# harukaki/brl

Hardware: AMD Instinct MI355X
Metric: env-steps/sec at num_envs=8192, 32-step rollout, 1/2/4/8 MI355X (higher is better)
Workload: dtype u8; 1 GPU; configs[1]: num_envs=8192 num_steps=32 random-policy rollout + DDS reward (fused kernel) + last_obs + GAE scan; num_envs_per_gpu=8192, num_steps=32, lut_len=100000, env_steps_per_macro_step=1, transition_buffers_in_rotation=3, device_warmup=3328 untimed steps (80 ms) before the --warmup steps: steady-state clocks, parallelism=env-shard x1, no collective

## Files before the change

brl_amd/build.py:

```python
from __future__ import annotations

import os
import shutil
import subprocess
import sys

PKG = os.path.dirname(os.path.abspath(__file__))
INCLUDE = os.path.join(os.path.dirname(PKG), "include")
OUT = os.path.join(PKG, "lib", "libbrl_hip.so")
OBJ_DIR = os.path.join(PKG, "lib", "obj")

FLAGS = ["--offload-arch=gfx950", "-O3", "-ffp-contract=off", "-fPIC", "-std=c++17"]


def units():
    import glob
    return sorted(glob.glob(os.path.join(PKG, "csrc", "*.hip")))


def headers():
    import glob
    return sorted(glob.glob(os.path.join(PKG, "csrc", "*.hpp")) + glob.glob(os.path.join(INCLUDE, "*.h")))


def deps():
    return units() + headers()


def hipcc() -> str:
    for cand in (os.environ.get("HIPCC"), shutil.which("hipcc"), "/opt/rocm/bin/hipcc"):
        if cand and os.path.exists(cand):
            return cand
    raise RuntimeError("hipcc not found (set HIPCC)")


def needs_build() -> bool:
    if not os.path.exists(OUT):
        return True
    t = os.path.getmtime(OUT)
    return any(os.path.getmtime(d) > t for d in deps())


def build(force: bool = False, verbose: bool = False) -> str:
    if not (force or needs_build()):
        return OUT
    os.makedirs(OBJ_DIR, exist_ok=True)
    newest_header = max(os.path.getmtime(h) for h in headers())
    procs, objs = [], []
    for src in units():
        obj = os.path.join(OBJ_DIR, os.path.splitext(os.path.basename(src))[0] + ".o")
        objs.append(obj)
        if force or not os.path.exists(obj) or os.path.getmtime(obj) < max(os.path.getmtime(src), newest_header):
            cmd = [hipcc()] + FLAGS + ["-c", "-o", obj, src]
            if verbose:
                print(" ".join(cmd), flush=True)
            procs.append((cmd, subprocess.Popen(cmd)))
    for cmd, p in procs:
        if p.wait() != 0:
            raise subprocess.CalledProcessError(p.returncode, cmd)
    cmd = [hipcc(), "--offload-arch=gfx950", "-shared", "-fPIC", "-o", OUT] + objs
    if verbose:
        print(" ".join(cmd), flush=True)
    subprocess.check_call(cmd)
    return OUT


if __name__ == "__main__":
    print(build(force="--force" in sys.argv, verbose=True))
```

brl_amd/csrc/brl_rollout.hip:

```cpp
#include <hip/hip_runtime.h>
#include <math.h>
#include <stdint.h>
#include <stdio.h>
#include <stdlib.h>
#include <string.h>

#include "handle.hpp"
#include "policy_common.hpp"

struct RolloutArgs {
  uint64_t *state;
  int64_t n;
  int T;
  int substeps;
  uint32_t draw_base;
  float reward_scale;
  Rng g;
  uint64_t env_offset;
  LutRef lut;
  const float *neg_log_n;
  brl_transition out;
  uint8_t *last_obs;
  uint8_t *last_mask;
  unsigned long long *terminated_count;
// ... 795 lines not shown
    };
#pragma unroll
    for (int u = 0; u < HGP; u++) {
      if (wv + 4 * u >= hsteps) break;
#pragma unroll
      for (int nb = 0; nb < 3; nb++) acc[nb] = mma(hav[u], hbok[nb] ? hbv[u][nb] : zero8, acc[nb]);
    }
    if (hsteps > 4 * HGP) {
      const int64_t row0 = xcd_block((int64_t)blockIdx.x, (int64_t)gridDim.x) * 16;
      const int64_t arow = (row0 + r < A.n) ? row0 + r : A.n - 1;
      const uint16_t *ap = reinterpret_cast<const uint16_t *>(A.x.head_h) + arow * A.x.head_ldh + 8 * kq;
      for (int st = wv + 4 * HGP; st < hsteps; st += 4) {
        const pol_b16x8 a = *reinterpret_cast<const pol_b16x8 *>(ap + 32 * st);
#pragma unroll
        for (int nb = 0; nb < 3; nb++) {
          const pol_b16x8 b = *reinterpret_cast<const pol_b16x8 *>(reinterpret_cast<const uint16_t *>(A.x.head_w) +
                                                                   (int64_t)(hbok[nb] ? 16 * nb + r : 0) * A.x.head_hidden + 8 * kq + 32 * st);
          acc[nb] = mma(a, hbok[nb] ? b : zero8, acc[nb]);
        }
      }
    }
#pragma unroll
    for (int nb = 0; nb < 3; nb++)
#pragma unroll
      for (int q = 0; q < 4; q++) hd_red[wv][nb][q][lane] = acc[nb][q];
    __syncthreads();
    for (int e = tid; e < 16 * POL_HD; e += BLOCK_THREADS) {
      const int row = e / POL_HD, col = e - row * POL_HD;
      const int nb = col >> 4, c = col & 15, q = row & 3, rq = row >> 2;
      float v = A.x.head_b[col];
#pragma unroll
      for (int k = 0; k < 4; k++) v += hd_red[k][nb][q][16 * rq + c];
      hd_logits[row][col] = v;
    }
    __syncthreads();
  }
  const DevCtx cx = *A.ctx;
  const uint64_t legal = legal_mask(t);
  const uint64_t cand = (A.mode & 2) ? ALL_ACTIONS : legal;
  const bool owner = w.c.lane < K && w.valid;
  const int64_t otab = owner ? w.table : 0;
  float4 old_rw = make_float4(0.f, 0.f, 0.f, 0.f);
  uint32_t old_term = 0, val_raw = 0, actor_id = 0;
  if (A.o.rewards && !A.x.first) old_rw = reinterpret_cast<const float4 *>(A.o.rewards)[otab];
  if (A.o.terminated && !A.x.first) old_term = A.o.terminated[otab];
  const int in_fmt = HEADS ? 0 : A.x.in_fmt;
  if (A.x.value_out) {
    if (HEADS) val_raw = __float_as_uint(hd_logits[(int)(threadIdx.x >> 6) * K + (w.c.lane < K ? w.c.lane : 0)][BRL_NUM_ACTIONS]);
    else if (A.x.in_fmt == 0) val_raw = reinterpret_cast<const uint32_t *>(A.x.value_in)[otab * A.x.value_stride];
    else val_raw = reinterpret_cast<const uint16_t *>(A.x.value_in)[otab * A.x.value_stride];
  }
  if (A.x.last && A.x.reward_out) actor_id = (uint32_t)A.x.actor[otab];
  uint32_t u32 = 0;
  if (!(A.mode & 1)) {
    uint32_t r[4];
    const uint64_t env_id = cx.env_offset + (uint64_t)w.table;
    const uint32_t draw = A.draw + (A.draw_dev ? *A.draw_dev : 0u);
    philox4x32_10((uint32_t)env_id, draw >> 2, STREAM_ACTION, (uint32_t)(env_id >> 32), cx.g.k0, cx.g.k1, r);
    u32 = philox_word(r, draw);
  }
  float lp;
  const int act = HEADS ? categorical<K>(&hd_logits[0][0], (int64_t)((int)(threadIdx.x >> 6) * K + w.tl) * (POL_HD + 1), 0, w.valid, cand,
                                         A.mode, u32, w.c.lane, lp)
                        : categorical<K>(A.logits, (w.valid ? w.table : 0) * A.logits_stride, A.x.in_fmt, w.valid, cand, A.mode, u32,
                                         w.c.lane, lp);
  if (A.autoreset) auto_reset_clear(t);
  int hb = table_step(t, act);
  wave_or_hist<K>(w, hb);
  wave_lds_fence();
  uint32_t term = bits(t.sc, SC_TERM, 1);
  float4 rw = rewards_f32(t);
  if (A.autoreset) wave_reset<K>(w, t, w.valid && term, cx.g, cx.env_offset, cx.lut, t.bctr + 1u);
  int oseat = cur_seat(t);
  wave_emit<K>(w, A.n, oseat, vul_nibble(t, oseat), legal_mask(t), A.o.obs, A.o.mask, w.table0);
  if (A.x.obs_cast != nullptr) {
    const uint32_t pack = (uint32_t)oseat | (vul_nibble(t, oseat) << 2);
    const int esz = (A.x.obs_fmt == 0) ? 4 : 2;
#pragma unroll
    for (int j = 0; j < K; j++) {
      if (w.table0 + j < A.n) {
        const uint32_t p = __builtin_amdgcn_readlane(pack, j);
        emit_obs_row_cast(w.wimg + j * TABLE_BYTES, (int)(p & 3u), p >> 2,
                          reinterpret_cast<uint8_t *>(A.x.obs_cast) + (w.table0 + j) * BRL_OBS_SIZE * esz, A.x.obs_fmt, w.c);
      }
    }
  }
  uint32_t tacc = 0;
  if (w.c.lane < K && w.valid) {
    if (A.action) A.action[w.table] = act;
    if (A.log_prob) A.log_prob[w.table] = lp;
    float4 tot = rw;
    if (A.o.rewards) {
      if (!A.x.first) tot = make_float4(old_rw.x + rw.x, old_rw.y + rw.y, old_rw.z + rw.z, old_rw.w + rw.w);
      reinterpret_cast<float4 *>(A.o.rewards)[w.table] = tot;
    }
    tacc = term;
    if (A.o.terminated) {
      if (!A.x.first) tacc |= old_term;
      A.o.terminated[w.table] = (uint8_t)tacc;
    }
    if (A.o.current_player) A.o.current_player[w.table] = cur_player(t);
    if (A.x.value_out) A.x.value_out[w.table] = net_cvt(val_raw, in_fmt);
    if (A.x.last) {
      if (A.x.done_out) A.x.done_out[w.table] = (uint8_t)tacc;
      if (A.x.reward_out) {
        const int a = (int)(actor_id & 3u);
        const float r = (a == 0) ? tot.x : ((a == 1) ? tot.y : ((a == 2) ? tot.z : tot.w));
        A.x.reward_out[w.table] = r / A.x.reward_scale;
      }
    }
  }
  if (A.x.last && A.x.terminated_count) {
    __shared__ uint32_t tc_s[WAVES_PER_BLOCK];
    const uint64_t m = __ballot(tacc != 0u);
    if (w.c.lane == 0) tc_s[threadIdx.x >> 6] = (uint32_t)__popcll(m);
    __syncthreads();
    if (threadIdx.x == 0) {
      uint32_t c = 0;
#pragma unroll
      for (int k = 0; k < WAVES_PER_BLOCK; k++) c += tc_s[k];
      if (c) atomicAdd(reinterpret_cast<unsigned long long *>(A.x.terminated_count), (unsigned long long)c);
    }
  }
  wave_end<K>(w, t, A.state_out, A.n);
}

static inline bool aligned_to(const void *p, uintptr_t a) { return ((uintptr_t)p & (a - 1)) == 0; }
static bool transition_aligned(const brl_transition *o, const void *last_obs, const void *last_mask, const void *adv, const void *tgt) {
  return aligned_to(o->obs, 16) && aligned_to(o->legal_action_mask, 16) && aligned_to(o->action, 16) && aligned_to(o->value, 16) &&
         aligned_to(o->reward, 16) && aligned_to(o->log_prob, 16) && aligned_to(o->done, 4) && aligned_to(last_obs, 16) &&
         aligned_to(last_mask, 16) && aligned_to(adv, 16) && aligned_to(tgt, 16);
}

static bool every_column(const brl_transition *o) {
  return o->obs && o->legal_action_mask && o->done && o->action && o->value && o->reward && o->log_prob;
}
static RolloutArgs rollout_args(brl_handle *h, uint64_t *state, int64_t n, int num_steps, int substeps, uint32_t draw_base,
                                float reward_scale, const brl_transition *out, uint8_t *last_obs, uint8_t *last_mask,
                                int64_t *terminated_count) {
  RolloutArgs A;
  A.state = state; A.n = n; A.T = num_steps; A.substeps = substeps; A.draw_base = draw_base;
  A.reward_scale = reward_scale; A.g = rng_of(h); A.env_offset = h->env_offset; A.lut = lut_of(h);
  A.neg_log_n = h->neg_log_n; A.out = *out; A.terminated_count = (unsigned long long *)terminated_count;
  A.last_obs = last_obs; A.last_mask = last_mask;
  A.gae_last_val = nullptr; A.gae_gamma = 0.0f; A.gae_gamma_lambda = 0.0f; A.gae_adv = nullptr; A.gae_tgt = nullptr;
#ifdef BRL_TIMING
  A.debug = getenv("BRL_DEBUG") ? atoi(getenv("BRL_DEBUG")) : 0;
#else
  A.debug = 0;
#endif
  return A;
}

extern "C" int brl_rollout_random(brl_handle *h, uint64_t *state, int64_t n, int num_steps, int substeps,
                                  uint32_t draw_base, float reward_scale, const brl_transition *out,
                                  uint8_t *last_obs, uint8_t *last_mask, int64_t *terminated_count, void *stream) {
  COMMON(h, n);
  NEED(state && out, "state / out");
  NEED(aligned_to(state, 16) && transition_aligned(out, last_obs, last_mask, nullptr, nullptr),
       "output arrays must be 16-byte aligned (done: 4-byte)");
  NEED(num_steps >= 0, "num_steps");
  NEED(substeps >= 1 && substeps <= 16, "substeps");
  if (h->lut_len == 0) return fail(BRL_E_NOLUT, "brl_rollout_random auto-resets and needs a LUT%s", "");
  const RolloutArgs A = rollout_args(h, state, n, num_steps, substeps, draw_base, reward_scale, out, last_obs, last_mask, terminated_count);
  if (h->ws && h->fs && substeps == 1 && n % FS_TPB == 0 && every_column(out)) {
    const int pieces = (num_steps + FS_MAX_TOTAL - 1) / FS_MAX_TOTAL;
    int t0 = 0;
    for (int i = 0; i < pieces || (pieces == 0 && i == 0); i++) {
      const int len = (pieces > 0) ? (num_steps - t0 + (pieces - i) - 1) / (pieces - i) : 0;
      const int64_t rows = (int64_t)t0 * n;
      RolloutArgs P = A;
      P.T = len;
      P.draw_base = draw_base + (uint32_t)t0;
      P.out.obs = out->obs + rows * BRL_OBS_SIZE;
      P.out.legal_action_mask = out->legal_action_mask + rows * BRL_NUM_ACTIONS;
      P.out.done = out->done + rows;
      P.out.action = out->action + rows;
      P.out.value = out->value + rows;
      P.out.reward = out->reward + rows;
      P.out.log_prob = out->log_prob + rows;
      const bool last = (i + 1 >= pieces);
      P.last_obs = last ? last_obs : nullptr;
      P.last_mask = last ? last_mask : nullptr;
      hipLaunchKernelGGL(k_rollout_fs, dim3((unsigned)(n / FS_TPB)), dim3(FS_NW * 64), 0, (hipStream_t)stream, P);
      t0 += len;
    }
  } else if (h->ws && substeps <= WS_BATCH) {
    hipLaunchKernelGGL((k_rollout_ws<32, 12, 1>), dim3((unsigned)((n + 31) / 32)), dim3(12 * 64), 0, (hipStream_t)stream, A);
  } else {
    LAUNCH_K(h, k_rollout_random, n, stream, A);
    return BRL_OK;
  }
  HIP_TRY(hipGetLastError());
  return BRL_OK;
}

extern "C" int brl_rollout_random_gae(brl_handle *h, uint64_t *state, int64_t n, int num_steps, uint32_t draw_base,
                                      float reward_scale, const brl_transition *out, uint8_t *last_obs, uint8_t *last_mask,
                                      int64_t *terminated_count, const float *last_val, float gamma, float gamma_lambda,
                                      float *advantages, float *targets, void *stream) {
  COMMON(h, n);
  NEED(state && out && last_val && advantages && targets, "state / out / last_val / advantages / targets");
  NEED(num_steps >= 1, "num_steps");
  NEED(out->done && out->value && out->reward, "the done / value / reward columns");
  NEED(aligned_to(state, 16) && transition_aligned(out, last_obs, last_mask, advantages, targets),
       "output arrays must be 16-byte aligned (done: 4-byte)");
  if (h->lut_len == 0) return fail(BRL_E_NOLUT, "brl_rollout_random_gae auto-resets and needs a LUT%s", "");
  if (!(h->ws && h->fs && num_steps <= FS_MAX_TOTAL && n % FS_TPB == 0 && every_column(out))) {
    const int rc = brl_rollout_random(h, state, n, num_steps, 1, draw_base, reward_scale, out, last_obs, last_mask,
                                      terminated_count, stream);
    if (rc != BRL_OK) return rc;
    return brl_gae(h, out->done, out->value, out->reward, last_val, gamma, gamma_lambda, num_steps, n, advantages, targets, stream);
  }
  RolloutArgs A = rollout_args(h, state, n, num_steps, 1, draw_base, reward_scale, out, last_obs, last_mask, terminated_count);
  A.gae_last_val = last_val; A.gae_gamma = gamma; A.gae_gamma_lambda = gamma_lambda; A.gae_adv = advantages; A.gae_tgt = targets;
  hipLaunchKernelGGL(k_rollout_fs, dim3((unsigned)(n / FS_TPB)), dim3(FS_NW * 64), 0, (hipStream_t)stream, A);
  HIP_TRY(hipGetLastError());
  return BRL_OK;
}

static int policy_step_impl(brl_handle *h, const uint64_t *state_in, uint64_t *state_out, int64_t n,
                            const float *logits, int64_t logits_stride, int mode, const uint32_t *draw_dev, uint32_t draw,
                            int autoreset,
                            int32_t *action, float *log_prob, uint8_t *obs, uint8_t *mask, float *rewards_acc,
                            uint8_t *terminated_acc, int32_t *current_player, void *stream, const brl_macro_ext *ext = nullptr) {
  NEED(step_outputs_aligned(state_in, state_out, obs, rewards_acc, action, current_player) && ptr_aligned(log_prob, 4) &&
           ptr_aligned(draw_dev, 4), STEP_ALIGN_MSG);
  NEED(ext == nullptr || (ptr_aligned(ext->obs_cast, 16) && ptr_aligned(ext->value_out, 4) && ptr_aligned(ext->reward_out, 4) &&
                          ptr_aligned(ext->actor, 4) && ptr_aligned(ext->terminated_count, 8)),
       "ext: obs_cast not 16-byte aligned (value_out / reward_out / actor: 4-byte, terminated_count: 8-byte)");
  COMMON(h, n);
  const bool heads = ext != nullptr && (ext->head_h != nullptr || ext->head_part != nullptr);
  NEED(state_in && state_out && (logits || heads), "NULL state / logits");
  NEED(mode >= 0 && mode <= 3, "mode");
  NEED(heads || logits_stride >= BRL_NUM_ACTIONS, "logits_stride");
  if (autoreset && h->lut_len == 0) return fail(BRL_E_NOLUT, "auto-reset needs a LUT%s", "");
  PolicyArgs A;
  A.state_in = state_in; A.state_out = state_out; A.n = n; A.logits = logits; A.mode = mode; A.draw = draw;
  A.logits_stride = logits_stride;
  A.draw_dev = draw_dev;
  A.autoreset = autoreset; A.ctx = h->ctx_dev;
  A.action = action; A.log_prob = log_prob;
  A.o = StepOut{obs, mask, rewards_acc, terminated_acc, current_player};
  memset(&A.x, 0, sizeof(A.x));
  if (ext != nullptr) {
    A.x = *ext;
    NEED(!ext->value_out || heads || (ext->value_in && ext->value_stride >= 1), "ext: value_in / value_stride");
    NEED(!ext->last || !ext->reward_out || (ext->actor && rewards_acc && ext->reward_scale != 0.0f), "ext: reward_out needs actor, rewards_acc, reward_scale");
    NEED(!ext->last || !(ext->done_out || ext->terminated_count) || terminated_acc, "ext: done_out / terminated_count need terminated_acc");
    NEED(!ext->obs_cast || (ext->obs_fmt >= 0 && ext->obs_fmt <= 2), "ext: obs_fmt");
    NEED(ext->in_fmt >= 0 && ext->in_fmt <= 2, "ext: in_fmt");
    if (ext->head_part != nullptr) {
      NEED(ext->head_b && ext->head_nparts >= 1 && ext->head_part_ld >= BRL_NUM_ACTIONS + 1 && ext->head_part_stride >= n * ext->head_part_ld,
           "ext: head_b / head_nparts / head_part_ld (>= 39) / head_part_stride (>= n * head_part_ld)");
      NEED(h->tables_per_wave == 4, "ext: head_part needs BRL_TABLES_PER_WAVE=4 (the head tile is a workgroup's 16 tables)");
      hipLaunchKernelGGL((k_policy_step<4, 2>), dim3(wave_grid(n, 4)), dim3(BLOCK_THREADS), 0, (hipStream_t)stream, A);
      HIP_TRY(hipGetLastError());
      return BRL_OK;
    }
    if (heads) {
      NEED(ext->head_w && ext->head_b && (ext->head_fmt == 1 || ext->head_fmt == 2), "ext: head_w / head_b / head_fmt (1 bf16, 2 fp16)");
      NEED(ext->head_hidden > 0 && ext->head_hidden % 32 == 0 && ext->head_ldh >= ext->head_hidden && ext->head_ldh % 8 == 0,
           "ext: head_hidden (a multiple of 32) / head_ldh (a multiple of 8)");
      NEED(h->tables_per_wave == 4, "ext: head_h needs BRL_TABLES_PER_WAVE=4 (the head tile is a workgroup's 16 tables)");
      hipLaunchKernelGGL((k_policy_step<4, 1>), dim3(wave_grid(n, 4)), dim3(BLOCK_THREADS), 0, (hipStream_t)stream, A);
      HIP_TRY(hipGetLastError());
      return BRL_OK;
    }
  }
  LAUNCH_K(h, k_policy_step, n, stream, A);
  return BRL_OK;
}

extern "C" int brl_policy_step(brl_handle *h, const uint64_t *state_in, uint64_t *state_out, int64_t n,
                               const float *logits, int mode, uint32_t draw, int autoreset, int32_t *action,
                               float *log_prob, uint8_t *obs, uint8_t *mask, float *rewards_acc,
                               uint8_t *terminated_acc, int32_t *current_player, void *stream) {
  return policy_step_impl(h, state_in, state_out, n, logits, BRL_NUM_ACTIONS, mode, nullptr, draw, autoreset, action,
                          log_prob, obs, mask, rewards_acc, terminated_acc, current_player, stream);
}

extern "C" int brl_policy_step_at(brl_handle *h, const uint64_t *state_in, uint64_t *state_out, int64_t n,
                                  const float *logits, int64_t logits_stride, int mode, const uint32_t *draw_base,
                                  uint32_t draw_offset, int autoreset, int32_t *action, float *log_prob, uint8_t *obs,
                                  uint8_t *mask, float *rewards_acc, uint8_t *terminated_acc, int32_t *current_player,
                                  void *stream) {
  return policy_step_impl(h, state_in, state_out, n, logits, logits_stride, mode, draw_base, draw_offset, autoreset,
                          action, log_prob, obs, mask, rewards_acc, terminated_acc, current_player, stream);
}

extern "C" int brl_policy_step_ex(brl_handle *h, const uint64_t *state_in, uint64_t *state_out, int64_t n,
                                  const float *logits, int64_t logits_stride, int mode, const uint32_t *draw_base,
                                  uint32_t draw_offset, int autoreset, int32_t *action, float *log_prob, uint8_t *obs,
                                  uint8_t *mask, float *rewards_acc, uint8_t *terminated_acc, int32_t *current_player,
                                  const brl_macro_ext *ext, void *stream) {
  return policy_step_impl(h, state_in, state_out, n, logits, logits_stride, mode, draw_base, draw_offset, autoreset,
                          action, log_prob, obs, mask, rewards_acc, terminated_acc, current_player, stream, ext);
}
```

brl_amd/csrc/rollout_fs.hpp:

```cpp
#pragma once

constexpr int FS_TPB = 32;
constexpr int FS_NW = 13;
constexpr int FS_MAX_TOTAL = 40;
#ifndef FS_RING_N
#define FS_RING_N 12
#endif
constexpr int FS_RING = FS_RING_N;
constexpr int FS_CHUNK = 8;
#ifndef FS_EXP
#define FS_EXP 0
#endif

typedef __attribute__((address_space(3))) volatile int fs_lds_int;
__device__ __forceinline__ int fs_flag_read(const int *p) {
  int v = *(fs_lds_int *)p;
  asm volatile("" ::: "memory");
  return __builtin_amdgcn_readfirstlane(v);
}
__device__ __forceinline__ void fs_flag_write(int *p, int v) {
  asm volatile("" ::: "memory");
  *(fs_lds_int *)p = v;
}
__device__ __forceinline__ void fs_wait(const int *flag, int s, int &avail) {
  if (s < avail) return;
  for (;;) {
    avail = fs_flag_read(flag);
    if (s < avail) return;
    __builtin_amdgcn_s_sleep(1);
  }
}

#ifdef BRL_TIMING
#define FS_STAMP(k) do { if (c.lane == 0 && A.terminated_count) fs_dump[2 * (k)] = __builtin_amdgcn_s_memtime() - t_begin; } while (0)
#else
#define FS_STAMP(k) do { } while (0)
#endif

__global__ __launch_bounds__(FS_NW * 64) void k_rollout_fs(RolloutArgs A) {
  constexpr int TPB = FS_TPB, NW = FS_NW;
#ifdef BRL_TIMING
  const unsigned long long t_begin = __builtin_amdgcn_s_memtime();
  const unsigned long long rt_begin = __builtin_amdgcn_s_memrealtime();
  unsigned long long t_wait = 0;
#endif
  __shared__ __attribute__((aligned(16))) uint8_t img[TPB * TABLE_BYTES];
  __shared__ __attribute__((aligned(16))) uint32_t cmd[FS_MAX_TOTAL + 1][TPB][CMD_WORDS];
  __shared__ __attribute__((aligned(16))) uint32_t ring[TPB][FS_RING][RING_WORDS];
  __shared__ uint32_t udraw[FS_MAX_TOTAL + 4][TPB];
  __shared__ float s_neglog[BRL_NUM_ACTIONS + 2];
  __shared__ __attribute__((aligned(16))) uint32_t raw[FS_MAX_TOTAL + 1][TPB][4];
  __shared__ int posted, raw_posted, ring_count, gae_ready;
  __shared__ __attribute__((aligned(16))) uint32_t oimg[TPB][4][16];
  __shared__ __attribute__((aligned(16))) uint32_t evq[FS_RING * TPB][4];
  __shared__ __attribute__((aligned(16))) uint32_t minfo_s[8 + FS_MAX_TOTAL][TPB];
  __shared__ __attribute__((aligned(16))) float frew_s[8 + FS_MAX_TOTAL][TPB];
  uint32_t(*const minfo)[TPB] = minfo_s + 8;
  float(*const frew)[TPB] = frew_s + 8;
  __shared__ __attribute__((aligned(16))) uint32_t last_rw[TPB][4];
  __shared__ int scored, ev_count;

  const int tid = (int)threadIdx.x;
  const int hw_wave = __builtin_amdgcn_readfirstlane(tid >> 6);
  constexpr uint64_t ROLE_OF_HW = 0x0ull | (3ull << 4) | (4ull << 8) | (1ull << 12) | (12ull << 16) | (5ull << 20) | (6ull << 24) |
                                  (7ull << 28) | (2ull << 32) | (8ull << 36) | (9ull << 40) | (10ull << 44) | (11ull << 48);
  const int wave = (int)((ROLE_OF_HW >> (4 * hw_wave)) & 15ull);
  const LaneConst c = make_lane_const();
#ifdef BRL_TIMING
  unsigned long long *fs_dump = A.terminated_count + (size_t)gridDim.x * NW * 2 + ((size_t)blockIdx.x * NW + wave) * 32;
#endif
  const int64_t table0 = xcd_block((int64_t)blockIdx.x, (int64_t)gridDim.x) * TPB;
  const int total = A.T;
  uint64_t *img64 = reinterpret_cast<uint64_t *>(img);
  static_assert(TPB * 16 <= NW * 64 && TPB * 64 <= 3 * NW * 64, "one table word and <= 3 image dwords per thread");
  const uint64_t st_word = (tid < TPB * 16) ? A.state[table0 * 16 + tid] : 0ull;
  const int lt = c.lane & (TPB - 1);
  uint64_t ctr_word = 0;
  if (wave == 1) ctr_word = A.state[(table0 + lt) * 16 + W_CTR];
  uint32_t oi_a[3], oi_sc[3];
  uint64_t oi_h[3];
  {
    const uint32_t *st32 = reinterpret_cast<const uint32_t *>(A.state + table0 * 16);
#pragma unroll
    for (int k = 0; k < 3; k++) {
      const int task = tid + k * NW * 64;
      const int tk = (task < TPB * 64) ? task : 0;
      const int t = tk >> 6, o = (tk >> 4) & 3, q = tk & 15;
      oi_a[k] = st32[t * 32 + ((q < 13) ? q : 13)];
      oi_h[k] = A.state[(table0 + t) * 16 + W_HAND + o];
      oi_sc[k] = st32[t * 32 + 2 * W_SC];
    }
  }
  const float neglog_v = (tid <= BRL_NUM_ACTIONS) ? A.neg_log_n[tid] : 0.0f;
  for (int i = tid; i < FS_MAX_TOTAL * TPB; i += NW * 64) (&frew[0][0])[i] = 0.0f;
  if (tid < TPB * 4) (&last_rw[0][0])[tid] = 0u;
  if (tid == 0) {
    posted = 0;
    raw_posted = 0;
    ring_count = 0;
    gae_ready = 0;
    scored = 0;
    ev_count = 0;
  }
  constexpr int LP = FS_RING / 2;
  brl_u32x4 ld_ha[LP], ld_hb[LP], ld_v[LP];
  uint32_t ld_idx[LP], ld_scb[LP];
  const int ld_half = c.lane >> 5;
  auto ld_issue = [&](int i) {
    const uint64_t eid = A.env_offset + (uint64_t)(table0 + lt);
    const uint32_t nb0 = (uint32_t)(ctr_word >> 32) + 1u;
    board_fetch(A.g, eid, nb0 + (uint32_t)(2 * i + ld_half), A.lut, ld_ha[i], ld_hb[i], ld_v[i], ld_idx[i], ld_scb[i]);
  };
  auto ld_commit = [&](int i) {
    board_commit(&ring[lt][2 * i + ld_half][0], ld_ha[i], ld_hb[i], ld_v[i], ld_idx[i], ld_scb[i]);
    if (c.lane == 0) fs_flag_write(&ring_count, 2 * i + 2);
  };
  if (wave == 1) {
    ld_issue(0);
    ld_issue(1);
  }
  {
    const uint32_t fb = A.draw_base >> 2;
    const int nblk = (total > 0) ? (int)(((A.draw_base & 3u) + (uint32_t)total + 3u) >> 2) : 0;
    for (int task = (hw_wave >= 4) ? tid - 4 * 64 : TPB * nblk; task < TPB * nblk; task += (NW - 4) * 64) {
      const int tb = task & (TPB - 1);
      const uint32_t blk = (fb + (uint32_t)(task >> 5)) & 0x3FFFFFFFu;
      const uint64_t eid = A.env_offset + (uint64_t)(table0 + tb);
      uint32_t rb[4];
      philox4x32_10((uint32_t)eid, blk, STREAM_ACTION, (uint32_t)(eid >> 32), A.g.k0, A.g.k1, rb);
#pragma unroll
      for (int k = 0; k < 4; k++) {
        const uint32_t s = ((blk << 2) | (uint32_t)k) - A.draw_base;
        if (s < (uint32_t)total) udraw[s][tb] = rb[k];
      }
    }
  }
  FS_STAMP(9);
  if (tid < TPB * 16) img64[tid] = st_word;
  FS_STAMP(10);
#pragma unroll
  for (int k = 0; k < 3; k++) {
    const int task = tid + k * NW * 64;
    if (task < TPB * 64) {
      const int t = task >> 6, o = (task >> 4) & 3, q = task & 15;
      const uint32_t a = oi_a[k];
      const uint64_t H = oi_h[k];
      const uint32_t m16 = __umul24(0xFu >> o, 0x1111u), m1 = m16 | (m16 << 16);
      const uint32_t rot = ((a >> o) & m1) | ((a << (4 - o)) & ~m1);
      uint32_t v = (q < 13) ? rot : ((q == 13) ? ((rot & 0xFFFu) | (uint32_t)(H << 8)) : ((q == 14) ? (uint32_t)(H >> 24) : 0u));
      v |= (q == 0) ? vul_nibble_sc(oi_sc[k], o) : 0u;
      oimg[t][o][q] = v;
    }
  }
  if (tid <= BRL_NUM_ACTIONS) s_neglog[tid] = neglog_v;
  FS_STAMP(11);
  __syncthreads();
  FS_STAMP(12);

  if (wave == 0) {
    const int tl = lt;
    uint32_t sc, sch, lut, bctr;
    {
      const uint2 *p = reinterpret_cast<const uint2 *>(img + tl * TABLE_BYTES);
      uint2 a = p[W_SC], d = p[W_CTR];
      sc = a.x; sch = a.y; lut = d.x; bctr = d.y;
    }
    __builtin_amdgcn_s_setprio(3);
    uint2 nxt = make_uint2(0u, 0u);
    bool have_nxt = false;
    int ring_seen = 0, kub = 0;
    uint32_t kt = 0;
    uint32_t pa = 0, psc = 0;
    uint32_t un = udraw[0][tl];
    for (int s = 0;; s++) {
      if (c.lane < TPB) *reinterpret_cast<uint4 *>(&raw[s][tl][0]) = make_uint4(sc, sch, pa, psc);
      if (c.lane == 0) fs_flag_write(&raw_posted, s + 1);
      if ((s & 7) == 0) FS_STAMP(s >> 3);
      if (s == 1 || s == 2) FS_STAMP(12 + s);
      if (s == total) break;
      const uint32_t u = un;
      un = udraw[(s + 2 < total) ? s + 1 : total - 1][tl];
      const uint32_t seat = lean_seat(sc, sch), lb1 = bits(sc, SC_LB1, 6);
      const uint32_t a = lean_pick(sc, seat, lb1, u);
      const uint32_t term = lean_apply(sc, sch, a, seat, lb1);
      psc = sc;
      pa = a | (term << 8) | (kt << 16);
      if (__any(term != 0u)) {
        kub++;
        const int need = (kub + 1 < FS_RING) ? kub + 1 : FS_RING;
        while (ring_seen < need) {
          ring_seen = fs_flag_read(&ring_count);
          if (ring_seen < need) __builtin_amdgcn_s_sleep(1);
        }
        if (!have_nxt) {
          nxt = *reinterpret_cast<const uint2 *>(&ring[tl][0][12]);
          have_nxt = true;
        }
        if (term) {
          sc = nxt.y | (sc & ((1u << SC_TERM) | (1u << SC_ILLEGAL)));
          sch = 0;
          lut = nxt.x;
          bctr += 1u;
          kt += 1u;
          nxt = *reinterpret_cast<const uint2 *>(&ring[tl][(kt < FS_RING) ? kt : FS_RING - 1][12]);
        }
      }
    }
    if (c.lane < TPB) {
      uint2 *p = reinterpret_cast<uint2 *>(img + tl * TABLE_BYTES);
      p[W_CTR] = make_uint2(lut, bctr);
    }
    if (A.gae_adv != nullptr) {
      const float gae_lv = A.gae_last_val[table0 + lt];
      while (fs_flag_read(&gae_ready) == 0) __builtin_amdgcn_s_sleep(1);
      FS_STAMP(5);
      if (c.lane < TPB) {
        float gae = 0.0f, next_value = gae_lv;
        const float g0 = A.gae_gamma * 0.0f;
        for (int t1 = total; t1 > 0; t1 -= 8) {
          float rr[8];
          uint32_t mi[8];
#pragma unroll
          for (int k = 0; k < 8; k++) {
            rr[k] = frew[t1 - 1 - k][lt];
            mi[k] = minfo[t1 - 1 - k][lt];
          }
#pragma unroll
          for (int k = 0; k < 8; k++) {
            const float nd = info_done(mi[k]) ? 0.0f : 1.0f;
            const float gnv = (k == 0 && t1 == total) ? A.gae_gamma * next_value : g0;
            const float delta = rr[k] + gnv * nd - 0.0f;
            gae = delta + A.gae_gamma_lambda * nd * gae;
            frew[t1 - 1 - k][lt] = gae;
          }
        }
      }
      FS_STAMP(6);
      wave_lds_order();
      const int q = c.lane >> 3, t4 = 4 * (c.lane & 7);
      for (int t = q; t < total; t += 8) {
        const int64_t i = (int64_t)t * A.n + table0 + t4;
        const float4 a = *reinterpret_cast<const float4 *>(&frew[t][t4]);
        const float4 b = make_float4(a.x + 0.0f, a.y + 0.0f, a.z + 0.0f, a.w + 0.0f);
        store_wt16(A.gae_adv + i, brl_u32x4{__float_as_uint(a.x), __float_as_uint(a.y), __float_as_uint(a.z), __float_as_uint(a.w)});
        store_wt16(A.gae_tgt + i, brl_u32x4{__float_as_uint(b.x), __float_as_uint(b.y), __float_as_uint(b.z), __float_as_uint(b.w)});
      }
    }
  } else if (wave == 12) {
    int avail = 0;
    int s = 0;
    while (s <= total) {
      fs_wait(&raw_posted, s, avail);
      const bool two = (s + 1 < avail);
      const int ms = s + ((two && c.lane >= TPB) ? 1 : 0);
      if (two || c.lane < TPB) {
        const uint4 cur = *reinterpret_cast<const uint4 *>(&raw[ms][lt][0]);
        const uint2 prv = *reinterpret_cast<const uint2 *>(&raw[(ms > 0) ? ms - 1 : 0][lt][0]);
        const uint32_t seat = lean_seat(cur.x, cur.y);
        uint32_t nl_cur, nl_prv;
        const uint64_t legal = lean_legal(cur.x, seat, nl_cur);
        const uint32_t seatp = lean_seat(prv.x, prv.y);
        (void)lean_legal(prv.x, seatp, nl_prv);
        const uint32_t a = cur.z & 63u;
        const uint32_t hb1 = lean_hb1(bits(prv.x, SC_LB1, 6), seatp, a);
        uint32_t pend = cmd_pack_prev(hb1, (cur.z >> 8) & 1u, (cur.z >> 16) & 15u, seatp, nl_prv);
        pend = (ms > 0) ? pend : 0u;
        const uint32_t w0 = cmd_pack_w0(pend, seat, 0u);
        *reinterpret_cast<uint4 *>(&cmd[ms][lt][0]) = make_uint4(w0, cur.w, (uint32_t)legal, cmd_pack_w3(legal, a));
      }
#ifdef BRL_TIMING
      if (s == 0) FS_STAMP(0);
      if (s < 2 && s + (two ? 2 : 1) >= 2) FS_STAMP(13);
      if (s < 3 && s + (two ? 2 : 1) >= 3) FS_STAMP(14);
#endif
      s += two ? 2 : 1;
      if (c.lane == 0) fs_flag_write(&posted, s);
    }
  } else if (wave == 1) {
#pragma unroll
    for (int i = 0; i < LP; i++) {
      ld_commit(i);
      if (i + 2 < LP) ld_issue(i + 2);
    }
    FS_STAMP(8);
    const MaskChunk mc[2] = {make_mask_chunk((uint32_t)c.lane, TPB), make_mask_chunk((uint32_t)c.lane + 64u, TPB)};
    uint8_t *mrow = A.out.legal_action_mask + table0 * BRL_NUM_ACTIONS;
    const int64_t mstep = A.n * BRL_NUM_ACTIONS;
    int avail = 0;
    for (int s = 0; s <= total; s++) {
      fs_wait(&posted, s, avail);
      uint8_t *dstrow = (s < total) ? mrow : ((A.last_mask != nullptr) ? A.last_mask + table0 * BRL_NUM_ACTIONS : nullptr);
      mrow += mstep;
      if (dstrow == nullptr) continue;
      const uint32_t(*cs)[CMD_WORDS] = cmd[s];
#pragma unroll
      for (int q = 0; q < 2; q++) {
        if (q == 1 && c.lane >= 12) break;
        store_wt16(dstrow + 16 * (c.lane + 64 * q), mask_chunk_bytes(cs, mc[q]));
      }
    }
  } else if (wave == 2) {
    const int tl = lt;
    const bool mine = c.lane < TPB;
    Tbl ts;
    load_scalars(ts, img + tl * TABLE_BYTES);
    uint32_t vslot = NO_SLOT;
    int avail = 0, nev = 0;
    uint4 wn = make_uint4(0u, 0u, 0u, 0u);
    for (int s = 1; s <= total; s++) {
      if (s >= avail) {
        fs_wait(&posted, s, avail);
        wn = *reinterpret_cast<const uint4 *>(&cmd[s][tl][0]);
      }
      const uint4 w = wn;
      if (s + 1 < avail) wn = *reinterpret_cast<const uint4 *>(&cmd[s + 1][tl][0]);
      const uint32_t info = scorer_follow(ts, vslot, nev, w, mine, (uint32_t)(s - 1), (uint32_t)tl, evq);
      if (mine) {
        minfo[s - 1][tl] = info;
        if (s == total) *reinterpret_cast<uint2 *>(&last_rw[tl][0]) = make_uint2(ts.fd, vslot);
      }
      if (c.lane == 0) {
        fs_flag_write(&ev_count, nev);
        fs_flag_write(&scored, s);
      }
      if ((s & 7) == 0) FS_STAMP(s >> 3);
    }
  } else if (wave == 11) {
    const int tl = lt;
    uint32_t tcount = 0;
    int b0 = 0, seen = 0, ev_done = 0;
    while (b0 < total) {
      fs_wait(&scored, b0, seen);
      const int evs = fs_flag_read(&ev_count);
      const int c1 = (seen < b0 + FS_CHUNK) ? seen : b0 + FS_CHUNK;
      const int m = c1 - b0;
      for (int e0 = ev_done; e0 < evs; e0 += 64) {
        const int e = e0 + c.lane;
        if (e < evs) {
          const uint4 q = *reinterpret_cast<const uint4 *>(&evq[e][0]);
          const uint32_t tt = ev_table(q), sl = ev_step(q);
          const Tbl tb = score_finished_board(q, ring[tt], img + tt * TABLE_BYTES);
          const int actor = (int)info_actor(minfo[sl][tt]);
          frew[sl][tt] = (float)reward_of(tb, actor) / A.reward_scale;
          if ((int)sl == total - 1) *reinterpret_cast<uint2 *>(&last_rw[tt][2]) = make_uint2(tb.r01, tb.r23);
        }
      }
      ev_done = evs;
      wave_lds_order();
      {
        const int q = c.lane >> 3, t4 = 4 * (c.lane & 7);
        uint4 info4 = make_uint4(0u, 0u, 0u, 0u);
        float4 rew = make_float4(0.f, 0.f, 0.f, 0.f);
        if (q < m) {
          info4 = *reinterpret_cast<const uint4 *>(&minfo[b0 + q][t4]);
          rew = *reinterpret_cast<const float4 *>(&frew[b0 + q][t4]);
        }
        wave_lds_order();
        if (A.gae_adv != nullptr && c1 == total && c.lane == 0) fs_flag_write(&gae_ready, 1);
        if (q < m) {
          brl_u32x4 act;
          float4 lgp;
          uint32_t dn;
          tcount += unpack_info4(info4, s_neglog, act, lgp, dn);
          const int64_t rw = (int64_t)(b0 + q) * A.n + table0 + t4;
          store_wt16(A.out.action + rw, act);
          store_wt16(A.out.value + rw, brl_u32x4{0u, 0u, 0u, 0u});
          store_wt16(A.out.reward + rw, brl_u32x4{__float_as_uint(rew.x), __float_as_uint(rew.y), __float_as_uint(rew.z), __float_as_uint(rew.w)});
          store_wt16(A.out.log_prob + rw, brl_u32x4{__float_as_uint(lgp.x), __float_as_uint(lgp.y), __float_as_uint(lgp.z), __float_as_uint(lgp.w)});
          *reinterpret_cast<uint32_t *>(A.out.done + rw) = dn;
        }
      }
      b0 = c1;
      if ((b0 & 7) == 0) FS_STAMP(b0 >> 3);
    }
    if (A.gae_adv != nullptr && total == 0 && c.lane == 0) fs_flag_write(&gae_ready, 1);
    add_terminated(A.terminated_count, tcount, c.lane);
    if (total > 0 && c.lane < TPB) {
      const uint4 f = *reinterpret_cast<const uint4 *>(&last_rw[tl][0]);
      uint2 *p = reinterpret_cast<uint2 *>(img + tl * TABLE_BYTES);
      if (f.y != NO_SLOT) {
        Tbl tb;
        const uint4 vv = *reinterpret_cast<const uint4 *>(&ring[tl][f.y][8]);
        pack_tricks(tb, vv.x, vv.y, vv.z, vv.w);
        p[W_FD] = make_uint2(f.x, tb.t2);
        p[W_TR] = make_uint2(tb.t0, tb.t1);
      } else {
        p[W_FD] = make_uint2(f.x, p[W_FD].y);
      }
      p[W_REW] = make_uint2(f.z, f.w);
    }
  } else if (wave <= 10) {
    const int g = wave - 3;
    const int L = c.lane;
    const bool active = L < 60;
    const int pq = active ? (L >> 1) : 29;
    const int r = pq / 15, q = pq - 15 * r;
    const int half = L & 1;
    const int hl = (L < 30) ? L : L - 30;
    const bool head = active && hl < 8;
    const int hsel = head ? (hl >> 2) : 0;
    const uint32_t ho = (uint32_t)(hl & 3);
    uint8_t *og = reinterpret_cast<uint8_t *>(&oimg[4 * g][0][0]);
    uint32_t *oh = reinterpret_cast<uint32_t *>(og + ((r + 2 * hsel) * 4 + (int)ho) * 64);
    const int rd_off = r * 256 + q * 4 + half * 2;
    const int dl_o = active ? L / 15 : 3, dl_q = active ? L - 15 * (L / 15) : 15;
    uint8_t *optr = A.out.obs + (table0 + 4 * g) * BRL_OBS_SIZE + 16 * L;
    const int64_t ostep = A.n * BRL_OBS_SIZE;
    int avail = 0;
    for (int s = 0; s <= total; s++) {
#ifdef BRL_TIMING
      const unsigned long long tw0 = __builtin_amdgcn_s_memtime();
#endif
      uint32_t w0a, w0b;
      if (s == 0) {
        const uint2 sa = reinterpret_cast<const uint2 *>(img + (4 * g + r) * TABLE_BYTES)[W_SC];
        const uint2 sb = reinterpret_cast<const uint2 *>(img + (4 * g + r + 2) * TABLE_BYTES)[W_SC];
        w0a = cmd_pack_w0(0u, lean_seat(sa.x, sa.y), 0u);
        w0b = cmd_pack_w0(0u, lean_seat(sb.x, sb.y), 0u);
      } else {
        fs_wait(&posted, s, avail);
        w0a = cmd[s][4 * g + r][0];
        w0b = cmd[s][4 * g + r + 2][0];
      }
#ifdef BRL_TIMING
      t_wait += __builtin_amdgcn_s_memtime() - tw0;
      if ((s & 7) == 0) FS_STAMP(s >> 3);
#endif
      if (s == (total >> 1)) {
        if (hw_wave >= 8) __builtin_amdgcn_s_setprio(2);
        else if (hw_wave >= 4) __builtin_amdgcn_s_setprio(1);
      }
      const uint32_t wh = hsel ? w0b : w0a;
      if (head && !cmd_deal(wh) && cmd_hist_bit1(wh)) {
        const uint32_t hb = cmd_hist_bit1(wh) - 1u;
        const uint32_t bit = (hb & ~3u) | ((hb - ho) & 3u);
        atomicOr(oh + (bit >> 5), 1u << (bit & 31u));
      }
      uint64_t dealm = __ballot(head && ho == 0u && cmd_deal(wh));
      while (dealm) {
        const int l = __ffsll((unsigned long long)dealm) - 1;
        dealm &= dealm - 1ull;
        const int row = (l >= 30) ? 1 + ((l - 30) >> 2) * 2 : (l >> 2) * 2;
        const uint32_t wq = __builtin_amdgcn_readlane(wh, l);
        const uint32_t *re = &ring[4 * g + row][cmd_ring_slot(wq)][0];
        const uint64_t H = *reinterpret_cast<const uint64_t *>(re + 2 * dl_o);
        const uint32_t v = (dl_q == 0) ? vul_nibble_sc(re[13], dl_o)
                                       : ((dl_q == 13) ? (uint32_t)(H << 8) : ((dl_q == 14) ? (uint32_t)(H >> 24) : 0u));
        if (active) oimg[4 * g + row][dl_o][dl_q] = v;
      }
      wave_lds_order();
      const uint32_t v0 = *reinterpret_cast<const uint16_t *>(og + rd_off + (int)cmd_observer(w0a) * 64);
      const uint32_t v1 = *reinterpret_cast<const uint16_t *>(og + rd_off + 512 + (int)cmd_observer(w0b) * 64);
      uint8_t *dst = (s < total) ? optr : ((A.last_obs != nullptr) ? A.last_obs + (table0 + 4 * g) * BRL_OBS_SIZE + 16 * L : nullptr);
      optr += ostep;
      if (active && dst != nullptr) {
#pragma unroll
        for (int k = 0; k < 2; k++) {
          const uint32_t word = k ? v1 : v0;
          const brl_u32x4 d = {nibble_bytes(word & 0xFu), nibble_bytes((word >> 4) & 0xFu), nibble_bytes((word >> 8) & 0xFu),
                               nibble_bytes(word >> 12)};
          if (!(FS_EXP & 8)) __builtin_nontemporal_store(d, reinterpret_cast<brl_u32x4 *>(dst + 960 * k));
          else if (d.x == 0x12345678u) __builtin_nontemporal_store(d, reinterpret_cast<brl_u32x4 *>(dst + 960 * k));
        }
      }
      if (s < 2) FS_STAMP(13 + s);
    }
  }
#ifdef BRL_TIMING
  if (c.lane == 0 && A.terminated_count) {
    unsigned long long *d = A.terminated_count + ((size_t)blockIdx.x * NW + wave) * 2;
    d[0] = __builtin_amdgcn_s_memtime() - t_begin;
    d[1] = t_wait;
    fs_dump[30] = __builtin_amdgcn_s_memrealtime() - rt_begin;
  }
#endif
  __syncthreads();
  for (int i = tid; i < TPB * 16; i += NW * 64) {
    const int t = i >> 4, w = i & 15;
    uint64_t v;
    if (w < 7) {
      uint32_t lo = oimg[t][0][2 * w], hi = oimg[t][0][2 * w + 1];
      lo = (w == 0) ? (lo & ~0xFu) : lo;
      hi = (w == 6) ? (hi & 0xFFFu) : hi;
      v = (uint64_t)lo | ((uint64_t)hi << 32);
    } else if (w < 11) {
      const uint32_t d13 = oimg[t][w - 7][13], d14 = oimg[t][w - 7][14];
      v = ((uint64_t)d14 << 24) | (uint64_t)((d13 >> 8) & 0xFFFFF0u);
    } else if (w == W_SC) {
      v = *reinterpret_cast<const uint64_t *>(&raw[total][t][0]);
    } else {
      v = img64[i];
    }
    A.state[table0 * 16 + i] = v;
  }
}
```

Baseline: 10.85 billion env-steps/s.

## Split fused rollout kernel args into preloaded hot scalars and deferred cold struct

The fused rollout kernel now takes its hot scalar and pointer arguments as separate kernel parameters, and the build enables AMDGPU kernarg preloading so these arrive in SGPRs at wave launch. The cold output pointers are fetched with two explicit s_load_dwordx16 loads whose wait is deferred until after the initial state loads. This is meant to shorten the kernel prologue's dependence on kernarg memory loads. In exchange it hardcodes kernarg byte offsets in inline asm, which is fragile if the argument layout or the compiler's preload behaviour changes.

```diff
diff --git a/brl_amd/build.py b/brl_amd/build.py
--- a/brl_amd/build.py
+++ b/brl_amd/build.py
@@ -11,6 +11,7 @@
 OBJ_DIR = os.path.join(PKG, "lib", "obj")
 
 FLAGS = ["--offload-arch=gfx950", "-O3", "-ffp-contract=off", "-fPIC", "-std=c++17"]
+UNIT_FLAGS = {"brl_rollout.hip": ["-mllvm", "-amdgpu-kernarg-preload-count=14", "-DFS_ARGS_PRELOADED"]}
 
 
 def units():
@@ -51,7 +52,7 @@
         obj = os.path.join(OBJ_DIR, os.path.splitext(os.path.basename(src))[0] + ".o")
         objs.append(obj)
         if force or not os.path.exists(obj) or os.path.getmtime(obj) < max(os.path.getmtime(src), newest_header):
-            cmd = [hipcc()] + FLAGS + ["-c", "-o", obj, src]
+            cmd = [hipcc()] + FLAGS + UNIT_FLAGS.get(os.path.basename(src), []) + ["-c", "-o", obj, src]
             if verbose:
                 print(" ".join(cmd), flush=True)
             procs.append((cmd, subprocess.Popen(cmd)))
@@ -65,5 +66,21 @@
     return OUT
 
 
+def build_variant(out: str, extra=()) -> str:
+    obj_dir = out + ".obj"
+    os.makedirs(obj_dir, exist_ok=True)
+    procs, objs = [], []
+    for src in units():
+        objs.append(os.path.join(obj_dir, os.path.splitext(os.path.basename(src))[0] + ".o"))
+        cmd = [hipcc()] + FLAGS + UNIT_FLAGS.get(os.path.basename(src), []) + list(extra) + ["-c", "-o", objs[-1], src]
+        procs.append((cmd, subprocess.Popen(cmd, stderr=subprocess.DEVNULL)))
+    for cmd, p in procs:
+        if p.wait() != 0:
+            raise subprocess.CalledProcessError(p.returncode, cmd)
+    subprocess.check_call([hipcc(), "--offload-arch=gfx950", "-shared", "-fPIC", "-o", out] + objs, stderr=subprocess.DEVNULL)
+    shutil.rmtree(obj_dir)
+    return out
+
+
 if __name__ == "__main__":
     print(build(force="--force" in sys.argv, verbose=True))
diff --git a/brl_amd/csrc/brl_rollout.hip b/brl_amd/csrc/brl_rollout.hip
--- a/brl_amd/csrc/brl_rollout.hip
+++ b/brl_amd/csrc/brl_rollout.hip
@@ -971,6 +971,16 @@
   return A;
 }
 
+static void launch_rollout_fs(const RolloutArgs &A, void *stream) {
+  FsColdArgs C;
+  C.reward_scale = A.reward_scale; C.gae_gamma = A.gae_gamma; C.gae_gamma_lambda = A.gae_gamma_lambda;
+  C.out = A.out; C.last_obs = A.last_obs; C.last_mask = A.last_mask; C.terminated_count = A.terminated_count;
+  C.gae_last_val = A.gae_last_val; C.gae_adv = A.gae_adv; C.gae_tgt = A.gae_tgt;
+  const unsigned nblocks = (unsigned)(A.n / FS_TPB);
+  hipLaunchKernelGGL(k_rollout_fs, dim3(nblocks), dim3(FS_NW * 64), 0, (hipStream_t)stream, A.state, A.env_offset, (uint32_t)nblocks,
+                     A.T, A.draw_base, A.g.k0, A.g.k1, A.lut.len, A.lut.hands, A.lut.values, A.neg_log_n, C);
+}
+
 extern "C" int brl_rollout_random(brl_handle *h, uint64_t *state, int64_t n, int num_steps, int substeps,
                                   uint32_t draw_base, float reward_scale, const brl_transition *out,
                                   uint8_t *last_obs, uint8_t *last_mask, int64_t *terminated_count, void *stream) {
@@ -1001,7 +1011,7 @@
       const bool last = (i + 1 >= pieces);
       P.last_obs = last ? last_obs : nullptr;
       P.last_mask = last ? last_mask : nullptr;
-      hipLaunchKernelGGL(k_rollout_fs, dim3((unsigned)(n / FS_TPB)), dim3(FS_NW * 64), 0, (hipStream_t)stream, P);
+      launch_rollout_fs(P, stream);
       t0 += len;
     }
   } else if (h->ws && substeps <= WS_BATCH) {
@@ -1033,7 +1043,7 @@
   }
   RolloutArgs A = rollout_args(h, state, n, num_steps, 1, draw_base, reward_scale, out, last_obs, last_mask, terminated_count);
   A.gae_last_val = last_val; A.gae_gamma = gamma; A.gae_gamma_lambda = gamma_lambda; A.gae_adv = advantages; A.gae_tgt = targets;
-  hipLaunchKernelGGL(k_rollout_fs, dim3((unsigned)(n / FS_TPB)), dim3(FS_NW * 64), 0, (hipStream_t)stream, A);
+  launch_rollout_fs(A, stream);
   HIP_TRY(hipGetLastError());
   return BRL_OK;
 }
diff --git a/brl_amd/csrc/rollout_fs.hpp b/brl_amd/csrc/rollout_fs.hpp
--- a/brl_amd/csrc/rollout_fs.hpp
+++ b/brl_amd/csrc/rollout_fs.hpp
@@ -37,13 +37,70 @@
 #define FS_STAMP(k) do { } while (0)
 #endif
 
-__global__ __launch_bounds__(FS_NW * 64) void k_rollout_fs(RolloutArgs A) {
+struct alignas(64) FsColdArgs {
+  brl_transition out;
+  uint8_t *last_obs;
+  uint8_t *last_mask;
+  unsigned long long *terminated_count;
+  const float *gae_last_val;
+  float *gae_adv, *gae_tgt;
+  float gae_gamma, gae_gamma_lambda;
+  float reward_scale;
+};
+#define FS_HOT_PARAMS                                                                                                  \
+  uint64_t *state_arg, uint64_t env_offset_arg, uint32_t nblocks_arg, int T_arg, uint32_t draw_base_arg, uint32_t k0_arg, \
+      uint32_t k1_arg, uint32_t lut_len_arg, const uint4 *lut_hands_arg, const int4 *lut_values_arg, const float *neg_log_n_arg
+template <class X>
+__device__ __forceinline__ X *fs_global(uint64_t bits) {
+  return (X *)(__attribute__((address_space(1))) X *)bits;
+}
+
+__global__ __launch_bounds__(FS_NW * 64) void k_rollout_fs(FS_HOT_PARAMS, FsColdArgs cold_arg) {
   constexpr int TPB = FS_TPB, NW = FS_NW;
 #ifdef BRL_TIMING
-  const unsigned long long t_begin = __builtin_amdgcn_s_memtime();
+  unsigned long long t_begin;
+  asm volatile("s_memtime %0\n\ts_waitcnt lgkmcnt(0)" : "=s"(t_begin));
   const unsigned long long rt_begin = __builtin_amdgcn_s_memrealtime();
   unsigned long long t_wait = 0;
 #endif
+  uint64_t env_offset = env_offset_arg;
+  uint32_t nblocks = nblocks_arg, draw_base = draw_base_arg, lut_len = lut_len_arg;
+  int total = T_arg;
+  Rng rng = {k0_arg, k1_arg};
+  uint64_t p_state = (uint64_t)state_arg, p_hands = (uint64_t)lut_hands_arg, p_values = (uint64_t)lut_values_arg;
+#ifdef FS_ARGS_PRELOADED
+  uint64_t p_neglog, p_obs, p_mask, p_done, p_action, p_value, p_reward, p_logp, p_lobs, p_lmask, p_tc, p_lv, p_adv, p_tgt;
+  uint32_t f_gamma, f_gl, f_rs;
+#else
+  uint64_t p_neglog = (uint64_t)neg_log_n_arg;
+  uint64_t p_obs = (uint64_t)cold_arg.out.obs, p_mask = (uint64_t)cold_arg.out.legal_action_mask, p_done = (uint64_t)cold_arg.out.done,
+           p_action = (uint64_t)cold_arg.out.action, p_value = (uint64_t)cold_arg.out.value, p_reward = (uint64_t)cold_arg.out.reward,
+           p_logp = (uint64_t)cold_arg.out.log_prob, p_lobs = (uint64_t)cold_arg.last_obs, p_lmask = (uint64_t)cold_arg.last_mask,
+           p_tc = (uint64_t)cold_arg.terminated_count, p_lv = (uint64_t)cold_arg.gae_last_val, p_adv = (uint64_t)cold_arg.gae_adv,
+           p_tgt = (uint64_t)cold_arg.gae_tgt;
+  uint32_t f_gamma = __float_as_uint(cold_arg.gae_gamma), f_gl = __float_as_uint(cold_arg.gae_gamma_lambda),
+           f_rs = __float_as_uint(cold_arg.reward_scale);
+#endif
+#define FS_PIN_HOT "+s"(p_state), "+s"(env_offset), "+s"(nblocks), "+s"(total), "+s"(draw_base), "+s"(rng.k0), "+s"(rng.k1), \
+                   "+s"(lut_len), "+s"(p_hands), "+s"(p_values)
+#define FS_PIN_REST "+s"(p_neglog), "+s"(p_obs), "+s"(p_mask), "+s"(p_done), "+s"(p_action), "+s"(p_value), "+s"(p_reward),     \
+                    "+s"(p_logp), "+s"(p_lobs), "+s"(p_lmask), "+s"(p_tc), "+s"(p_lv), "+s"(p_adv), "+s"(p_tgt), "+s"(f_gamma), \
+                    "+s"(f_gl), "+s"(f_rs)
+#ifdef FS_ARGS_PRELOADED
+  typedef uint32_t fs_u32x16 __attribute__((ext_vector_type(16)));
+  static_assert(sizeof(FsColdArgs) == 128 && offsetof(FsColdArgs, reward_scale) == 112, "r_a, r_b: kernarg bytes 0x38..0xb8");
+  fs_u32x16 r_a, r_b;
+  asm volatile("s_load_dwordx16 %0, %2, 0x38\n\ts_load_dwordx16 %1, %2, 0x78"
+               : "=&s"(r_a), "=&s"(r_b) : "s"(__builtin_amdgcn_kernarg_segment_ptr()));
+  asm volatile("" : FS_PIN_HOT);
+#else
+  asm volatile("" : FS_PIN_HOT, FS_PIN_REST);
+#endif
+#ifdef BRL_TIMING
+  const unsigned long long t_args = __builtin_amdgcn_s_memtime();
+#endif
+  uint64_t *const state = fs_global<uint64_t>(p_state);
+  const LutRef lut = {nullptr, fs_global<const int4>(p_values), lut_len, fs_global<const uint4>(p_hands)};
   __shared__ __attribute__((aligned(16))) uint8_t img[TPB * TABLE_BYTES];
   __shared__ __attribute__((aligned(16))) uint32_t cmd[FS_MAX_TOTAL + 1][TPB][CMD_WORDS];
   __shared__ __attribute__((aligned(16))) uint32_t ring[TPB][FS_RING][RING_WORDS];
@@ -66,32 +123,61 @@
                                   (7ull << 28) | (2ull << 32) | (8ull << 36) | (9ull << 40) | (10ull << 44) | (11ull << 48);
   const int wave = (int)((ROLE_OF_HW >> (4 * hw_wave)) & 15ull);
   const LaneConst c = make_lane_const();
-#ifdef BRL_TIMING
-  unsigned long long *fs_dump = A.terminated_count + (size_t)gridDim.x * NW * 2 + ((size_t)blockIdx.x * NW + wave) * 32;
-#endif
-  const int64_t table0 = xcd_block((int64_t)blockIdx.x, (int64_t)gridDim.x) * TPB;
-  const int total = A.T;
+  const int64_t table0 = xcd_block((int64_t)blockIdx.x, (int64_t)nblocks) * TPB;
+  const int64_t n = (int64_t)nblocks * TPB;
   uint64_t *img64 = reinterpret_cast<uint64_t *>(img);
   static_assert(TPB * 16 <= NW * 64 && TPB * 64 <= 3 * NW * 64, "one table word and <= 3 image dwords per thread");
-  const uint64_t st_word = (tid < TPB * 16) ? A.state[table0 * 16 + tid] : 0ull;
+  const uint64_t st_word = (tid < TPB * 16) ? state[table0 * 16 + tid] : 0ull;
   const int lt = c.lane & (TPB - 1);
   uint64_t ctr_word = 0;
-  if (wave == 1) ctr_word = A.state[(table0 + lt) * 16 + W_CTR];
+  if (wave == 1) ctr_word = state[(table0 + lt) * 16 + W_CTR];
   uint32_t oi_a[3], oi_sc[3];
   uint64_t oi_h[3];
   {
-    const uint32_t *st32 = reinterpret_cast<const uint32_t *>(A.state + table0 * 16);
+    const uint32_t *st32 = reinterpret_cast<const uint32_t *>(state + table0 * 16);
 #pragma unroll
     for (int k = 0; k < 3; k++) {
       const int task = tid + k * NW * 64;
       const int tk = (task < TPB * 64) ? task : 0;
       const int t = tk >> 6, o = (tk >> 4) & 3, q = tk & 15;
       oi_a[k] = st32[t * 32 + ((q < 13) ? q : 13)];
-      oi_h[k] = A.state[(table0 + t) * 16 + W_HAND + o];
+      oi_h[k] = state[(table0 + t) * 16 + W_HAND + o];
       oi_sc[k] = st32[t * 32 + 2 * W_SC];
     }
   }
-  const float neglog_v = (tid <= BRL_NUM_ACTIONS) ? A.neg_log_n[tid] : 0.0f;
+#ifdef FS_ARGS_PRELOADED
+  asm volatile("s_waitcnt lgkmcnt(0)" : "+s"(r_a), "+s"(r_b));
+#define FS_U64(v, i) ((uint64_t)(v)[i] | ((uint64_t)(v)[(i) + 1] << 32))
+  p_neglog = FS_U64(r_a, 0);
+  p_done = FS_U64(r_a, 2); p_action = FS_U64(r_a, 4); p_value = FS_U64(r_a, 6); p_reward = FS_U64(r_a, 8);
+  p_logp = FS_U64(r_a, 10); p_obs = FS_U64(r_a, 12); p_mask = FS_U64(r_a, 14);
+  p_lobs = FS_U64(r_b, 0); p_lmask = FS_U64(r_b, 2); p_tc = FS_U64(r_b, 4); p_lv = FS_U64(r_b, 6);
+  p_adv = FS_U64(r_b, 8); p_tgt = FS_U64(r_b, 10);
+  f_gamma = r_b[12]; f_gl = r_b[13]; f_rs = r_b[14];
+#undef FS_U64
+#endif
+  const float *const neg_log_n = fs_global<const float>(p_neglog);
+  const float neglog_v = (tid <= BRL_NUM_ACTIONS) ? neg_log_n[tid] : 0.0f;
+  FsColdArgs A;
+  A.out.obs = fs_global<uint8_t>(p_obs);
+  A.out.legal_action_mask = fs_global<uint8_t>(p_mask);
+  A.out.done = fs_global<uint8_t>(p_done);
+  A.out.action = fs_global<int32_t>(p_action);
+  A.out.value = fs_global<float>(p_value);
+  A.out.reward = fs_global<float>(p_reward);
+  A.out.log_prob = fs_global<float>(p_logp);
+  A.last_obs = fs_global<uint8_t>(p_lobs);
+  A.last_mask = fs_global<uint8_t>(p_lmask);
+  A.terminated_count = fs_global<unsigned long long>(p_tc);
+  A.gae_last_val = fs_global<const float>(p_lv);
+  A.gae_adv = fs_global<float>(p_adv);
+  A.gae_tgt = fs_global<float>(p_tgt);
+  A.gae_gamma = __uint_as_float(f_gamma);
+  A.gae_gamma_lambda = __uint_as_float(f_gl);
+  A.reward_scale = __uint_as_float(f_rs);
+#ifdef BRL_TIMING
+  unsigned long long *fs_dump = A.terminated_count + (size_t)nblocks * NW * 2 + ((size_t)blockIdx.x * NW + wave) * 32;
+#endif
   for (int i = tid; i < FS_MAX_TOTAL * TPB; i += NW * 64) (&frew[0][0])[i] = 0.0f;
   if (tid < TPB * 4) (&last_rw[0][0])[tid] = 0u;
   if (tid == 0) {
@@ -107,9 +193,9 @@
   uint32_t ld_idx[LP], ld_scb[LP];
   const int ld_half = c.lane >> 5;
   auto ld_issue = [&](int i) {
-    const uint64_t eid = A.env_offset + (uint64_t)(table0 + lt);
+    const uint64_t eid = env_offset + (uint64_t)(table0 + lt);
     const uint32_t nb0 = (uint32_t)(ctr_word >> 32) + 1u;
-    board_fetch(A.g, eid, nb0 + (uint32_t)(2 * i + ld_half), A.lut, ld_ha[i], ld_hb[i], ld_v[i], ld_idx[i], ld_scb[i]);
+    board_fetch(rng, eid, nb0 + (uint32_t)(2 * i + ld_half), lut, ld_ha[i], ld_hb[i], ld_v[i], ld_idx[i], ld_scb[i]);
   };
   auto ld_commit = [&](int i) {
     board_commit(&ring[lt][2 * i + ld_half][0], ld_ha[i], ld_hb[i], ld_v[i], ld_idx[i], ld_scb[i]);
@@ -120,17 +206,17 @@
     ld_issue(1);
   }
   {
-    const uint32_t fb = A.draw_base >> 2;
-    const int nblk = (total > 0) ? (int)(((A.draw_base & 3u) + (uint32_t)total + 3u) >> 2) : 0;
+    const uint32_t fb = draw_base >> 2;
+    const int nblk = (total > 0) ? (int)(((draw_base & 3u) + (uint32_t)total + 3u) >> 2) : 0;
     for (int task = (hw_wave >= 4) ? tid - 4 * 64 : TPB * nblk; task < TPB * nblk; task += (NW - 4) * 64) {
       const int tb = task & (TPB - 1);
       const uint32_t blk = (fb + (uint32_t)(task >> 5)) & 0x3FFFFFFFu;
-      const uint64_t eid = A.env_offset + (uint64_t)(table0 + tb);
+      const uint64_t eid = env_offset + (uint64_t)(table0 + tb);
       uint32_t rb[4];
-      philox4x32_10((uint32_t)eid, blk, STREAM_ACTION, (uint32_t)(eid >> 32), A.g.k0, A.g.k1, rb);
+      philox4x32_10((uint32_t)eid, blk, STREAM_ACTION, (uint32_t)(eid >> 32), rng.k0, rng.k1, rb);
 #pragma unroll
       for (int k = 0; k < 4; k++) {
-        const uint32_t s = ((blk << 2) | (uint32_t)k) - A.draw_base;
+        const uint32_t s = ((blk << 2) | (uint32_t)k) - draw_base;
         if (s < (uint32_t)total) udraw[s][tb] = rb[k];
       }
     }
@@ -239,7 +325,7 @@
       wave_lds_order();
       const int q = c.lane >> 3, t4 = 4 * (c.lane & 7);
       for (int t = q; t < total; t += 8) {
-        const int64_t i = (int64_t)t * A.n + table0 + t4;
+        const int64_t i = (int64_t)t * n + table0 + t4;
         const float4 a = *reinterpret_cast<const float4 *>(&frew[t][t4]);
         const float4 b = make_float4(a.x + 0.0f, a.y + 0.0f, a.z + 0.0f, a.w + 0.0f);
         store_wt16(A.gae_adv + i, brl_u32x4{__float_as_uint(a.x), __float_as_uint(a.y), __float_as_uint(a.z), __float_as_uint(a.w)});
@@ -285,7 +371,7 @@
     FS_STAMP(8);
     const MaskChunk mc[2] = {make_mask_chunk((uint32_t)c.lane, TPB), make_mask_chunk((uint32_t)c.lane + 64u, TPB)};
     uint8_t *mrow = A.out.legal_action_mask + table0 * BRL_NUM_ACTIONS;
-    const int64_t mstep = A.n * BRL_NUM_ACTIONS;
+    const int64_t mstep = n * BRL_NUM_ACTIONS;
     int avail = 0;
     for (int s = 0; s <= total; s++) {
       fs_wait(&posted, s, avail);
@@ -362,7 +448,7 @@
           float4 lgp;
           uint32_t dn;
           tcount += unpack_info4(info4, s_neglog, act, lgp, dn);
-          const int64_t rw = (int64_t)(b0 + q) * A.n + table0 + t4;
+          const int64_t rw = (int64_t)(b0 + q) * n + table0 + t4;
           store_wt16(A.out.action + rw, act);
           store_wt16(A.out.value + rw, brl_u32x4{0u, 0u, 0u, 0u});
           store_wt16(A.out.reward + rw, brl_u32x4{__float_as_uint(rew.x), __float_as_uint(rew.y), __float_as_uint(rew.z), __float_as_uint(rew.w)});
@@ -405,7 +491,7 @@
     const int rd_off = r * 256 + q * 4 + half * 2;
     const int dl_o = active ? L / 15 : 3, dl_q = active ? L - 15 * (L / 15) : 15;
     uint8_t *optr = A.out.obs + (table0 + 4 * g) * BRL_OBS_SIZE + 16 * L;
-    const int64_t ostep = A.n * BRL_OBS_SIZE;
+    const int64_t ostep = n * BRL_OBS_SIZE;
     int avail = 0;
     for (int s = 0; s <= total; s++) {
 #ifdef BRL_TIMING
@@ -472,6 +558,7 @@
     d[0] = __builtin_amdgcn_s_memtime() - t_begin;
     d[1] = t_wait;
     fs_dump[30] = __builtin_amdgcn_s_memrealtime() - rt_begin;
+    fs_dump[1] = t_args - t_begin;
   }
 #endif
   __syncthreads();
@@ -491,6 +578,6 @@
     } else {
       v = img64[i];
     }
-    A.state[table0 * 16 + i] = v;
+    state[table0 * 16 + i] = v;
   }
 }
```

Result: no change. 10.94 billion env-steps/s, median of 6 (+0.8%).
